# DeliriumV01D/NeRFpp

Measured on AMD Instinct MI355X. Metric: ray-samples/sec (HIP volume-rendering path, Lego 800x800, N_samples=64+128), higher is better.
Workload: dtype f16x3

## Files before the change

include/nerfpp_hip.h:

```cpp
#ifndef NERFPP_HIP_H
#define NERFPP_HIP_H

#include <stddef.h>
#include <stdint.h>

#ifdef __cplusplus
extern "C" {
#endif

#define NRF_API __attribute__((visibility("default")))

enum {
    NRF_OK = 0,
    NRF_ERR_INVALID_ARG = 1,
    NRF_ERR_HIP = 2,
    NRF_ERR_UNSUPPORTED = 3,
    NRF_ERR_WORKSPACE = 4,
    NRF_ERR_NONFINITE = 5
};

NRF_API int nrf_version(void);
NRF_API const char *nrf_last_error(void);
NRF_API const char *nrf_status_string(int status);

// ... 436 lines not shown
                                   void *d_workspace, size_t workspace_bytes, void *stream);
NRF_API size_t nrf_lerf_backward_points_workspace_bytes(const nrf_lerf_renderer *r, int64_t n, int s);
NRF_API int nrf_lerf_backward_points(const nrf_lerf_renderer *r, const float *d_pts, const float *d_z, const float *d_dirs, int d_stride, int64_t n, int s, const float *d_noise,
                                     float noise_std, const float *d_g_rendered, float *d_g_lerf_params, float *d_g_table, void *d_workspace, size_t workspace_bytes, void *stream);
NRF_API int nrf_lerf_renderer_last_features(const nrf_lerf_renderer *r, const void **d_feats_lm, int64_t *cols, const uint8_t **d_keep_cols, const int32_t **d_src, int64_t *n, int *sf,
                                            uint64_t *serial );
NRF_API int nrf_lerf_backward_points_src(const nrf_lerf_renderer *r, const void *d_feats_lm, int64_t cols, const uint8_t *d_keep_cols, const int32_t *d_src, const float *d_pts,
                                         const float *d_z, const float *d_dirs, int d_stride, int64_t n, int s, const float *d_noise, float noise_std, const float *d_g_rendered,
                                         float *d_g_lerf_params, float *d_g_table, void *d_workspace, size_t workspace_bytes, void *stream);

NRF_API size_t nrf_scratch_trim(void);

enum { NRF_PROF_HASH = 0, NRF_PROF_MLP = 1, NRF_PROF_COMPOSITE = 2, NRF_PROF_SAMPLE = 3, NRF_PROF_OTHER = 4, NRF_PROF_SIGMA = 5, NRF_PROF_MLP_COLOUR = 6, NRF_PROF_COUNT = 7 };
NRF_API int nrf_set_render_lanes(int lanes);
NRF_API int nrf_get_render_lanes(void);
NRF_API int nrf_renderer_set_lanes(nrf_renderer *r, int lanes);
NRF_API int nrf_fp32_gemm_available(void);
NRF_API int nrf_get_train_gemm(void);
NRF_API int nrf_set_train_gemm(int mode);
NRF_API int nrf_gemm_nt_bf16x3(const float *d_a, int lda, int64_t m, int k, const float *d_b, int ldb, int n, float *d_c, int ldc, const float *d_bias, int relu, void *stream);
NRF_API int nrf_gemm_tn_bf16x3(const float *d_g, int ldg, int out, const float *d_x, int ldx, int n, int64_t p, float *d_dw, int in, int col0, void *stream);
NRF_API int nrf_layer_grad_split(const float *d_g, int ldg, int out, const float *d_x, int ldx, int n, int64_t p, float *d_dw, int in, int col0, float *d_db, void *stream);
NRF_API int nrf_gemm_nt_f16x3(const float *d_a, int lda, int64_t m, int k, const float *d_b, int ldb, int n, float *d_c, int ldc, const float *d_bias, int relu, void *stream);
NRF_API int nrf_profile_enable(int on);
NRF_API int nrf_profile_is_enabled(void);
NRF_API int nrf_profile_read(double *ms , int64_t *launches , int reset);

#ifdef __cplusplus
}
#endif
// ... 2 lines not shown
```

nerfpp_amd/_lib.py:

```python
import ctypes as C
import os
import re

_HERE = os.path.dirname(os.path.abspath(__file__))
LIB_PATH = os.environ.get("NRF_LIB_PATH") or os.path.join(_HERE, "lib", "libnerfpp_hip.so")

NRF_OK = 0
NRF_HASH_NGP, NRF_HASH_CU = 0, 1
NRF_SH_LIBTORCH, NRF_SH_CUDA = 0, 1
NRF_PREC_F32, NRF_PREC_F16_MFMA, NRF_PREC_F16_SPLIT = 0, 1, 2
NRF_DIRS_NONE, NRF_DIRS_PE, NRF_DIRS_SH_LIBTORCH, NRF_DIRS_SH_CUDA = 0, 1, 2, 3
(NRF_RNG_T_RAND, NRF_RNG_R_COARSE, NRF_RNG_THETA_COARSE, NRF_RNG_NOISE_COARSE, NRF_RNG_U_PDF, NRF_RNG_PRECOND, NRF_RNG_R_FINE, NRF_RNG_THETA_FINE,
 NRF_RNG_NOISE_FINE) = range(1, 10)
NRF_PROF_NAMES = ("hash", "mlp", "composite", "sample", "other", "sigma", "mlp_colour")
NRF_COARSE_AUTO, NRF_COARSE_FULL, NRF_COARSE_SIGMA_F32 = 0, 1, 2
NRF_OVERFLOW_AUTO, NRF_OVERFLOW_RERENDER, NRF_OVERFLOW_ERROR, NRF_OVERFLOW_DEFERRED, NRF_OVERFLOW_IGNORE = 0, 1, 2, 3, 4
NRF_ERR_NONFINITE = 5
NRF_NORMALS_DENSITY, NRF_NORMALS_PREDICTED = 1, 2


class HashDesc(C.Structure):
    _fields_ = [("mode", C.c_int), ("n_levels", C.c_int), ("n_features", C.c_int), ("log2_hashmap_size", C.c_int),
                ("base_resolution", C.c_int), ("finest_resolution", C.c_int), ("bbox", C.c_float * 6)]

# ... 227 lines not shown
    nrf_lerf_head_relevancy(pplpipiiipppzp)
    nrf_lerf_point_relevancy_workspace_bytes(plil)->z
    nrf_lerf_point_relevancy(ppliipplpzp)
    nrf_lerf_relevancy_grid_workspace_bytes(piiiil)->z
    nrf_lerf_relevancy_grid(ppiiiiipplpzp)
    nrf_huber_rows_nanmean(pplifppp)
    nrf_lerf_head_backward_workspace_bytes(pli)->z
    nrf_lerf_head_backward(pppppilipfppppppzp)
    nrf_lerf_backward_points_workspace_bytes(pli)->z
    nrf_lerf_backward_points(ppppilipfppppzp)
    nrf_lerf_renderer_last_features(pppppppp)
    nrf_lerf_backward_points_src(pplpppppilipfppppzp)
    nrf_scratch_trim()->z
    nrf_set_render_lanes(i)
    nrf_get_render_lanes()
    nrf_renderer_set_lanes(pi)
    nrf_fp32_gemm_available()
    nrf_get_train_gemm()
    nrf_set_train_gemm(i)
    nrf_gemm_nt_bf16x3(pilipiipipip)
    nrf_gemm_tn_bf16x3(piipiilpiip)
    nrf_layer_grad_split(piipiilpiipp)
    nrf_gemm_nt_f16x3(pilipiipipip)
    nrf_profile_enable(i)
    nrf_profile_is_enabled()
    nrf_profile_read(ppi)
"""
SIGNATURES = {}
for _entry in _ABI.split():
    _m = re.fullmatch(r"(nrf_\w+)\(([ilzfduqp]*)\)(?:->([lzpsv]))?", _entry)
# ... 33 lines not shown
```

nerfpp_amd/csrc/mlp.h:

```cpp
#pragma once
#include "common.h"

#include <functional>
#include <vector>

namespace nrf {

enum { MLP_SMALL = 0, MLP_NERF = 1, MLP_LERF = 2 };

enum : uint8_t { WM_ZERO = 0, WM_F16_HI = 1, WM_F16_LO = 2, WM_F32 = 3 };
struct WeightMap {
    int32_t *d_src = nullptr;
    uint8_t *d_kind = nullptr;
    int64_t n = 0;
    int elem = 2;
    void *d_out = nullptr;
    bool scaled = false;
};

enum { SMALL_MAX_GROUPS = 12, SMALL_SCALE_INV_SIGMA = 0, SMALL_SCALE_INV_RGB = 1, SMALL_SCALE_HIDDEN = 2, SMALL_SCALE_COUNT = 8 };

struct LinearLayer {
    int in = 0, out = 0;
    float *d_wt = nullptr;
// ... 75 lines not shown
int train_gemm_mode();
int train_gemm_for(const nrf_mlp *m);
bool run_backprop_uses_mask_bits(const nrf_mlp *m, int64_t npts, int width);
bool gemm_nt_bits_ok(int64_t M, int N);
int gemm_nt_split(int arithmetic, int64_t M, int N, Seg a, Seg b, const float *B, int ldb, float *c, int ldc, const float *bias, int relu, const float *mask, int mask_ld,
                  hipStream_t st, const float *add = nullptr, int add_ld = 0, const float *r1s = nullptr, int r1s_ld = 0, const float *r1w = nullptr,
                  uint64_t *bits_out = nullptr, int bits_out_ld = 0, const uint64_t *bits_in = nullptr, int bits_in_ld = 0);
int gemm_rm(hipStream_t st, bool transA, bool transB, int64_t M, int64_t N, int64_t K, float alpha, const float *A, int lda, const float *B, int ldb, float beta, float *C, int ldc);

int mlp_small_mfma_available(const nrf_mlp *m);
int mlp_small_rescale(nrf_mlp *m, hipStream_t st);
int mlp_small_forward_mfma_lm(const nrf_mlp *m, const __half2 *feats, const __half2 *feats_lo, int64_t pstride, const __half *dirs, const __half *dirs_lo, int s,
                              const uint8_t *keep, int64_t p, float *out, hipStream_t st, const int32_t *src = nullptr);
int mlp_small_color_from_geo_lm(const nrf_mlp *m, const void *geo, int64_t geo_stride, const float *sigma, const __half *dirs, const __half *dirs_lo, int s,
                                const uint8_t *keep, int64_t p, float *out, hipStream_t st);
int mlp_small_pack_sigma_f32(nrf_mlp *m, const std::vector<float> &host_params);
int mlp_small_sigma_f32_available(const nrf_mlp *m);
int mlp_small_sigma_f32_lm(const nrf_mlp *m, const void *feats, int f32_in, int64_t pstride, const uint8_t *keep, int64_t p, float *sigma, hipStream_t st, void *geo = nullptr,
                           int64_t geo_stride = 0);
int mlp_nerf_mfma_available(const nrf_mlp *m);
int mlp_nerf_forward_mfma_fused(const nrf_mlp *m, const float *pts, const float *rays, int ray_stride, const float *z, int s, const __half *dirs, int64_t p, float *out, hipStream_t st);
int launch_dirs_pe_f16(const float *rays, int stride, int64_t n, __half *out, hipStream_t st);
int mlp_nerf_split_available(const nrf_mlp *m);
int mlp_nerf_forward_split_rows(const nrf_mlp *m, const float *x, int xs, int64_t p, float *out, int os, hipStream_t st);
int mlp_nerf_forward_split_fused(const nrf_mlp *m, const float *pts, const float *rays, int ray_stride, const float *z, int s, const __half *dirs, const __half *dirs_lo,
                                 int64_t p, float *out, hipStream_t st);
int launch_dirs_pe_split(const float *rays, int stride, int64_t n, __half *out_hi, __half *out_lo, hipStream_t st);
int mlp_small_pack_f16(nrf_mlp *m, const std::vector<float> &host_params);
int mlp_small_pack_bwd(nrf_mlp *m, const std::vector<float> &host_params);
bool mlp_small_images_host(const nrf_mlp_small_desc &d, const std::vector<float> &hp, std::vector<uint8_t> &f16_img, std::vector<uint8_t> &split_img);
// ... 25 lines not shown
```

nerfpp_amd/csrc/mlp_small_mfma.hip:

```cpp
#include "mfma_frag.h"
#include "mlp.h"

#include <type_traits>

namespace nrf {

typedef _Float16 half2v __attribute__((ext_vector_type(2)));

#ifdef NRF_SMALL_TRACE
__device__ unsigned long long g_small_trace[256 * 12];
#define NRF_TSTAMP(i) do { const unsigned long long t__ = __builtin_readcyclecounter(); tr[i] += t__ - tprev; tprev = t__; } while (0)
#else
#define NRF_TSTAMP(i) do { } while (0)
#endif
#ifndef NRF_SMALL_PT
#define NRF_SMALL_PT 2
#endif
constexpr int PT = NRF_SMALL_PT;
#ifndef NRF_SPLIT_WAVES
#define NRF_SPLIT_WAVES 8
#endif
#ifndef NRF_SPLIT_MINWAVES
#define NRF_SPLIT_MINWAVES 1
#endif
// ... 84 lines not shown
struct SmallPlan {
    static constexpr int GEO_KS = 1;
    static constexpr int sigma_frags(int l) { return (l == NL - 1 ? 1 : 2) * (l == 0 ? IN_KS : 4); }
    static constexpr int color_frags(int l) { return (l == NLC - 1 ? 1 : 2) * (l == 0 ? (V_KS + GEO_KS) : 4); }
    static constexpr int sigma_total() { int t = 0; for (int l = 0; l < NL; l++) t += sigma_frags(l); return t; }
    static constexpr int total()
    {
        int t = 0;
        for (int l = 0; l < NL; l++) t += sigma_frags(l);
        for (int l = 0; l < NLC; l++) t += color_frags(l);
        return t;
    }
};

struct SmallInput {
    const float *x; int x_stride; int in_ch;
    const __half2 *feats; int64_t pstride;
    const __half *dirs; int s;
    const uint8_t *keep;
    const __half *dirs_lo;
    const __half2 *feats_lo;
    const int32_t *src;
    const half8 *geo; int64_t geo_stride;
    const float *sigma;
    uint32_t ray_mul; int ray_shift;
    const float *scales;
};

#ifndef NRF_SMALL_PIPE_SPLIT
#define NRF_SMALL_PIPE_SPLIT 1
#endif
// ... 5 lines not shown
#endif
#ifndef NRF_SMALL_PREFETCH_F16
#define NRF_SMALL_PREFETCH_F16 0
#endif
#ifndef NRF_SMALL_STAGGER
#define NRF_SMALL_STAGGER 0
#endif
#ifndef NRF_SMALL_FINE
#define NRF_SMALL_FINE 1
#endif
#ifndef NRF_SMALL_DROP_MASK
#define NRF_SMALL_DROP_MASK 0
#endif
constexpr int small_drop_of(int id) { return (int)((((unsigned long long)NRF_SMALL_DROP_MASK) >> (2 * id)) & 3ull); }

template <int IN_KS, int V_KS, int NL, int NLC, bool LM, bool SPLIT, bool LMLO = false, bool GEOIN = false, bool A32 = false>
__global__ void __launch_bounds__(64 * waves_of(SPLIT), SPLIT ? NRF_SPLIT_MINWAVES : 2)
k_mlp_small_mfma(int64_t npts, SmallInput in, const half8 *__restrict__ packed, float *__restrict__ out, int out_stride)
{
    using Plan = SmallPlan<IN_KS, V_KS, NL, NLC>;
    constexpr int NP = SPLIT ? 2 : 1;
    constexpr int BLOCK_PTS = block_pts_of(SPLIT);
    constexpr bool IN_LO = SPLIT && (!LM || LMLO);
    static_assert(!GEOIN || (LM && SPLIT && !LMLO), "the colour-only kernel exists in split precision on the level-major path");
    extern __shared__ __attribute__((aligned(16))) unsigned char smem[];
    half8 *wl = reinterpret_cast<half8 *>(smem);
    constexpr int NFRAG = Plan::total() * NP;
    for (int i = threadIdx.x; i < NFRAG * 64; i += blockDim.x) wl[i] = packed[i];
    __syncthreads();

    const int lane = threadIdx.x & 63, wave = threadIdx.x >> 6;
    const int r = lane & 31, h = lane >> 5;
    const int64_t nblocks = (npts + BLOCK_PTS - 1) / BLOCK_PTS;
    float inv_sigma = 1.0f, inv_rgb = 1.0f;
    if constexpr (SPLIT) { inv_sigma = in.scales[SMALL_SCALE_INV_SIGMA]; inv_rgb = in.scales[SMALL_SCALE_INV_RGB]; }
    (void)inv_sigma; (void)inv_rgb;
#if NRF_SMALL_STAGGER
    if (SPLIT && wave >= 4) {
#pragma unroll
        for (int i = 0; i < NRF_SMALL_STAGGER; i++) __builtin_amdgcn_s_sleep(127);
    }
#endif
    auto split8 = [](const float4 &lo4, const float4 &hi4, half8 &hv, half8 &lv) {
        const float v[8] = {lo4.x, lo4.y, lo4.z, lo4.w, hi4.x, hi4.y, hi4.z, hi4.w};
#pragma unroll
        for (int j = 0; j < 8; j++) { const _Float16 t = (_Float16)v[j]; hv[j] = t; lv[j] = (_Float16)(v[j] - (float)t); }
    };
    static_assert(!A32 || (LM && SPLIT), "32-bit addressing is instantiated for the split-precision level-major kernels");
    auto load_cols = [&](int64_t blk_, int32_t (&cols)[PT]) {
        if (A32 || !(LM && in.src)) return;
        const int64_t p0_ = blk_ * BLOCK_PTS + wave * (32 * PT);
#pragma unroll
        for (int pt = 0; pt < PT; pt++) {
            int64_t p = p0_ + pt * 32 + r;
            if (p >= npts) p = npts - 1;
            cols[pt] = (LM && in.src) ? in.src[p] : (int32_t)0;
        }
    };
    auto load_inputs = [&](int64_t blk_, const int32_t (&cols)[PT], half8 (&bx)[PT][IN_KS][NP], half8 (&bv)[PT][V_KS][NP], uint8_t (&kpv)[PT], half8 (&bg)[PT][NP], float (&sgv)[PT]) {
        const int64_t p0_ = blk_ * BLOCK_PTS + wave * (32 * PT);
#pragma unroll
        for (int pt = 0; pt < PT; pt++) {
            int64_t p = p0_ + pt * 32 + r;
            if (p >= npts) p = npts - 1;
            kpv[pt] = 1;
            if constexpr (LM) {
                if constexpr (A32) {
                    uint32_t pu = (uint32_t)p0_ + (uint32_t)(pt * 32 + r);
                    pu = pu < (uint32_t)npts ? pu : (uint32_t)npts - 1u;
                    if (in.keep) kpv[pt] = in.keep[pu];
                    if constexpr (GEOIN) {
                        const uint32_t goff = (pu * 2u + (uint32_t)h) * 16u;
                        bg[pt][0] = *reinterpret_cast<const half8 *>(reinterpret_cast<const char *>(in.geo) + goff);
                        bg[pt][NP - 1] = *reinterpret_cast<const half8 *>(reinterpret_cast<const char *>(in.geo + in.geo_stride * 2) + goff);
                        sgv[pt] = in.sigma[pu];
                    } else {
                        const uint32_t voff = ((uint32_t)(4 * h) * (uint32_t)in.pstride + pu) * 4u;
#pragma unroll
                        for (int s = 0; s < IN_KS; s++) {
                            union { half8 v; __half2 q[4]; } u;
#pragma unroll
                            for (int q = 0; q < 4; q++) u.q[q] = *reinterpret_cast<const __half2 *>(reinterpret_cast<const char *>(in.feats + (int64_t)(8 * s + q) * in.pstride) + voff);
                            bx[pt][s][0] = u.v;
                            if constexpr (SPLIT && LMLO) {
#pragma unroll
// ... 45 lines not shown
                    const float4 hi = *reinterpret_cast<const float4 *>(row + 16 * s + 8 * h + 4);
                    if constexpr (SPLIT) split8(lo, hi, bx[pt][s][0], bx[pt][s][NP - 1]);
                    else bx[pt][s][0] = half8{(_Float16)lo.x, (_Float16)lo.y, (_Float16)lo.z, (_Float16)lo.w, (_Float16)hi.x, (_Float16)hi.y, (_Float16)hi.z, (_Float16)hi.w};
                }
#pragma unroll
                for (int s = 0; s < V_KS; s++) {
                    const float4 lo = *reinterpret_cast<const float4 *>(row + in.in_ch + 16 * s + 8 * h);
                    const float4 hi = *reinterpret_cast<const float4 *>(row + in.in_ch + 16 * s + 8 * h + 4);
                    if constexpr (SPLIT) split8(lo, hi, bv[pt][s][0], bv[pt][s][NP - 1]);
                    else bv[pt][s][0] = half8{(_Float16)lo.x, (_Float16)lo.y, (_Float16)lo.z, (_Float16)lo.w, (_Float16)hi.x, (_Float16)hi.y, (_Float16)hi.z, (_Float16)hi.w};
                }
            }
        }
    };
    constexpr bool PREFETCH = LM && (SPLIT ? (NRF_SMALL_PREFETCH_SPLIT != 0) : (NRF_SMALL_PREFETCH_F16 != 0));
    half8 bx[PT][IN_KS][NP];
    half8 bv[PT][V_KS][NP];
    half8 bxn[PREFETCH ? PT : 1][IN_KS][NP];
    half8 bvn[PREFETCH ? PT : 1][V_KS][NP];
    half8 bg[PT][NP], bgn[PT][NP];
    float sgv[PT], sgn[PT];
    (void)bg; (void)bgn; (void)sgv; (void)sgn;
    uint8_t kp[PT], kpn[PT];
    int32_t cols_next[PT];
#pragma unroll
    for (int pt = 0; pt < PT; pt++) { kp[pt] = 1; kpn[pt] = 1; cols_next[pt] = 0; }
    if constexpr (PREFETCH) {
        if ((int64_t)blockIdx.x < nblocks) {
            int32_t c0[PT];
            load_cols(blockIdx.x, c0);
            if ((int64_t)blockIdx.x + gridDim.x < nblocks) load_cols((int64_t)blockIdx.x + gridDim.x, cols_next);
            load_inputs(blockIdx.x, c0, bx, bv, kp, bg, sgv);
        }
    }
#ifdef NRF_SMALL_TRACE
    unsigned long long tr[12] = {0, 0, 0, 0, 0, 0, 0, 0, 0, 0, 0, 0};
#endif
    for (int64_t blk = blockIdx.x; blk < nblocks; blk += gridDim.x) {
#ifdef NRF_SMALL_TRACE
        const unsigned long long titer = __builtin_readcyclecounter();
        unsigned long long tprev = titer;
#endif
        const int64_t p0 = blk * BLOCK_PTS + wave * (32 * PT);
        if constexpr (!PREFETCH) { int32_t c0[PT]; load_cols(blk, c0); load_inputs(blk, c0, bx, bv, kp, bg, sgv); }
        const bool more = blk + gridDim.x < nblocks;
        const half8 *fr = wl;
        constexpr bool PIPE = SPLIT ? (NRF_SMALL_PIPE_SPLIT != 0) : (NRF_SMALL_PIPE_F16 != 0);
// ... 90 lines not shown
                                if (i >= i0 && i < i1) conv_item(bb, tt, i);
                        }
                    }
                }
            };
        };
        if constexpr (GEOIN) fr += Plan::sigma_total() * 64 * NP;
        half8 pre[NP];
#pragma unroll
        for (int q = 0; q < NP; q++) pre[q] = fr[q * 64 + lane];
        f32x16 sig[PT][1];
        auto prefetch_next = [&]() {
            if constexpr (PREFETCH) {
                if (more) {
                    load_inputs(blk + gridDim.x, cols_next, bxn, bvn, kpn, bgn, sgn);
                    if (blk + 2 * (int64_t)gridDim.x < nblocks) load_cols(blk + 2 * (int64_t)gridDim.x, cols_next);
                }
            }
        };
        if constexpr (GEOIN) {
        } else if constexpr (NL == 1) {
            gemm_layer<1, IN_KS, NP, IN_LO>(fr, lane, bx, sig, pre); fr += Plan::sigma_frags(0) * 64 * NP;
        } else {
            gemm_layer<2, IN_KS, NP, IN_LO, false, FINE, small_drop_of(0)>(fr, lane, bx, acc2, pre, make_job(1, false, true, IN_KS, std::true_type{}, std::bool_constant<!(small_drop_of(1) & 2)>{})); fr += Plan::sigma_frags(0) * 64 * NP;
            prefetch_next();
            NRF_TSTAMP(0);
            static_assert(NL <= 3, "sigma net: at most three layers");
            if constexpr (NL == 3) {
                if constexpr (!PIPE) hidden_to_b(0);
                gemm_layer<2, 4, NP, SPLIT, false, FINE, small_drop_of(1)>(fr, lane, bh[0], acc2, pre, make_job(0, true, true, 4, std::bool_constant<!(small_drop_of(1) & 2)>{}, std::bool_constant<!(small_drop_of(2) & 2)>{}));
// ... 42 lines not shown
                fr += Plan::color_frags(2) * 64 * NP;
                NRF_TSTAMP(6);
            }
            {
                constexpr int l = NLC - 1;
                const int bi = PIPE ? ((l - 1) & 1) : 0;
                if constexpr (!PIPE) hidden_to_b(0);
                gemm_layer<1, 4, NP, SPLIT, true, FINE, small_drop_of(NL + l)>(fr, lane, bh[bi], rgb, pre, make_job(bi, true, false, 4, std::bool_constant<!(small_drop_of(NL + l) & 2)>{}, std::true_type{}));
                fr += Plan::color_frags(l) * 64 * NP;
                NRF_TSTAMP(4 + l);
            }
        }
        if (h == 0) {
#pragma unroll
            for (int pt = 0; pt < PT; pt++) {
                const int64_t p = p0 + pt * 32 + r;
                if (p < npts) {
                    float sg;
                    if constexpr (GEOIN) sg = sgv[pt]; else if constexpr (SPLIT) sg = sig[pt][0][0] * inv_sigma; else sg = sig[pt][0][0];
                    if constexpr (LM) { if (!kp[pt]) sg = 0.0f; }
                    float c0 = rgb[pt][0][0], c1 = rgb[pt][0][1], c2 = rgb[pt][0][2];
                    if constexpr (SPLIT) { c0 *= inv_rgb; c1 *= inv_rgb; c2 *= inv_rgb; }
                    if (out_stride == 4) *reinterpret_cast<float4 *>(out + p * 4) = float4{c0, c1, c2, sg};
                    else { float *o = out + p * out_stride; o[0] = c0; o[1] = c1; o[2] = c2; o[3] = sg; }
                }
            }
        }
        if constexpr (PREFETCH) {
            if (more) {
#pragma unroll
                for (int pt = 0; pt < PT; pt++) {
#pragma unroll
                    for (int s = 0; s < IN_KS; s++)
#pragma unroll
                        for (int q = 0; q < NP; q++) bx[pt][s][q] = bxn[pt][s][q];
#pragma unroll
                    for (int s = 0; s < V_KS; s++)
#pragma unroll
                        for (int q = 0; q < NP; q++) bv[pt][s][q] = bvn[pt][s][q];
                    kp[pt] = kpn[pt];
                    if constexpr (GEOIN) { bg[pt][0] = bgn[pt][0]; bg[pt][NP - 1] = bgn[pt][NP - 1]; sgv[pt] = sgn[pt]; }
                }
            }
        }
#ifdef NRF_SMALL_TRACE
        NRF_TSTAMP(8);
        tr[9] += __builtin_readcyclecounter() - titer; tr[10] += 1;
#endif
    }
#ifdef NRF_SMALL_TRACE
    if (threadIdx.x == 0 && SPLIT && LM) for (int i = 0; i < 12; i++) g_small_trace[blockIdx.x * 12 + i] += tr[i];
#endif
}

#ifdef NRF_SMALL_TRACE
extern "C" NRF_API int nrf_dbg_small_trace(unsigned long long *host_out, int reset)
// ... 80 lines not shown
    if (!mlp_small_images_host(d, hp, a, b)) return NRF_OK;
    auto upload = [](void *&dst, size_t &have, const std::vector<uint8_t> &img) -> int {
        const size_t bytes = img.size();
        if (dst && have != bytes) { (void)hipFree(dst); dst = nullptr; }
        if (!dst) NRF_HIP(hipMalloc(&dst, bytes));
        have = bytes;
        NRF_HIP(hipMemcpy(dst, img.data(), bytes, hipMemcpyHostToDevice));
        return NRF_OK;
    };
    NRF_TRY(upload(m->d_packed_f16, m->packed_f16_bytes, a));
    NRF_TRY(upload(m->d_packed_split, m->packed_split_bytes, b));
    return mlp_small_pack_bwd(m, hp);
}

template <int V_KS, int NL, int NLC>
static int launch_small(const nrf_mlp *m, const SmallInput &in, bool lm, bool split, int64_t p, float *out, int os, hipStream_t st)
{
    using Plan = SmallPlan<2, V_KS, NL, NLC>;
    const size_t lds = (size_t)Plan::total() * 1024 * (split ? 2 : 1);
    const size_t have = split ? m->packed_split_bytes : m->packed_f16_bytes;
    if (lds != have) { set_error("internal: packed weight image is %zu bytes, kernel expects %zu", have, lds); return NRF_ERR_INVALID_ARG; }
    const int64_t nblocks = ceil_div(p, block_pts_of(split));
    const int64_t cap = split ? 256 : 768;
    const unsigned grid = (unsigned)(nblocks < cap ? nblocks : cap);
    const half8 *img = reinterpret_cast<const half8 *>(split ? m->d_packed_split : m->d_packed_f16);
#define NRF_GO(LM_, SP_, LO_, ...)                                                                                                            \
    do {                                                                                                                                      \
        auto kfn = k_mlp_small_mfma<2, V_KS, NL, NLC, LM_, SP_, LO_, ##__VA_ARGS__>;                                                          \
        if (lds > 64 * 1024) NRF_HIP(hipFuncSetAttribute(reinterpret_cast<const void *>(kfn), hipFuncAttributeMaxDynamicSharedMemorySize, (int)lds)); \
        hipLaunchKernelGGL(kfn, dim3(grid), dim3(64 * waves_of(SP_)), lds, st, p, in, img, out, os);                                          \
    } while (0)
    const bool a32 = lm && split && !in.src && (p >> 26) == 0 && (in.pstride >> 27) == 0 && (in.geo_stride >> 26) == 0 && in.ray_mul != 0 &&
                     (((uint64_t)(p / (in.s > 0 ? in.s : 1)) + 1) * (uint64_t)(32 * V_KS)) >> 32 == 0;
    if (in.geo) {
        if (!lm || !split) { set_error("internal: the colour-only NeRFSmall kernel is split precision, level-major"); return NRF_ERR_INVALID_ARG; }
        if (a32) NRF_GO(true, true, false, true, true); else NRF_GO(true, true, false, true);
    } else if (lm) {
        if (split) {
            if (in.feats_lo) { if (a32) NRF_GO(true, true, true, false, true); else NRF_GO(true, true, true); }
            else { if (a32) NRF_GO(true, true, false, false, true); else NRF_GO(true, true, false); }
        } else NRF_GO(true, false, false);
    }
    else { if (split) NRF_GO(false, true, false); else NRF_GO(false, false, false); }
#undef NRF_GO
    NRF_LAUNCH_CHECK();
    return NRF_OK;
}

static int dispatch_small(const nrf_mlp *m, const SmallInput &in, bool lm, bool split, int64_t p, float *out, int os, hipStream_t st);

int mlp_small_mfma_available(const nrf_mlp *m) { return m && m->family == MLP_SMALL && m->d_packed_f16 != nullptr && m->d_packed_split != nullptr; }

int mlp_small_forward_mfma_lm(const nrf_mlp *m, const __half2 *feats, const __half2 *feats_lo, int64_t pstride, const __half *dirs, const __half *dirs_lo, int s,
                              const uint8_t *keep, int64_t p, float *out, hipStream_t st, const int32_t *src)
{
    if (!mlp_small_mfma_available(m)) { set_error("internal: matrix-core NeRFSmall image missing"); return NRF_ERR_UNSUPPORTED; }
    ProfScope prof(NRF_PROF_MLP, st);
    SmallInput in{nullptr, 0, m->small.input_ch, feats, pstride, dirs, s, keep, dirs_lo, dirs_lo ? feats_lo : nullptr, src, nullptr, 0, nullptr};
    return dispatch_small(m, in, true, dirs_lo != nullptr, p, out, 4, st);
}

int mlp_small_color_from_geo_lm(const nrf_mlp *m, const void *geo, int64_t geo_stride, const float *sigma, const __half *dirs, const __half *dirs_lo, int s,
                                const uint8_t *keep, int64_t p, float *out, hipStream_t st)
{
    if (!mlp_small_mfma_available(m)) { set_error("internal: matrix-core NeRFSmall image missing"); return NRF_ERR_UNSUPPORTED; }
    if (!geo || !sigma || !dirs_lo) { set_error("internal: colour-only pass without geo planes / sigma / split direction features"); return NRF_ERR_INVALID_ARG; }
    ProfScope prof(NRF_PROF_MLP_COLOUR, st);
    SmallInput in{nullptr, 0, m->small.input_ch, nullptr, 0, dirs, s, keep, dirs_lo, nullptr, nullptr, static_cast<const half8 *>(geo), geo_stride, sigma};
    return dispatch_small(m, in, true, true, p, out, 4, st);
}

int mlp_small_forward_mfma(const nrf_mlp *m, const float *x, int xs, int64_t p, int split, float *out, int os, hipStream_t st)
{
    const auto &d = m->small;
    if (!m->d_packed_f16) {
        set_error("NRF_PREC_F16_MFMA / NRF_PREC_F16_SPLIT: NeRFSmall shape (in %d, views %d, %dx%d, geo %d, colour %dx%d) is outside the built matrix-core family; use NRF_PREC_F32",
                  d.input_ch, d.input_ch_views, d.num_layers, d.hidden_dim, d.geo_feat_dim, d.num_layers_color, d.hidden_dim_color);
        return NRF_ERR_UNSUPPORTED;
    }
    if ((xs % 4) != 0 || (reinterpret_cast<uintptr_t>(x) & 15)) { set_error("NRF_PREC_F16_MFMA: input rows must be 16-byte aligned"); return NRF_ERR_INVALID_ARG; }
    SmallInput in{x, xs, d.input_ch, nullptr, 0, nullptr, 1, nullptr, nullptr, nullptr, nullptr, nullptr, 0, nullptr};
    return dispatch_small(m, in, false, split != 0, p, out, os, st);
}

static int dispatch_small(const nrf_mlp *m, const SmallInput &in_, bool lm, bool split, int64_t p, float *out, int os, hipStream_t st)
{
    const auto &d = m->small;
    SmallInput in = in_;
    in.ray_mul = 0; in.ray_shift = 0;
    in.scales = m->d_scales;
    if (lm && in.s >= 1) {
        int L = 0;
        while ((1 << L) < in.s) L++;
        if (L == 0) { in.ray_mul = 1; in.ray_shift = -1; }
        else { in.ray_mul = (uint32_t)((((uint64_t)1 << (31 + L)) + (uint64_t)in.s - 1) / (uint64_t)in.s); in.ray_shift = L - 1; }
    }
    const int v = d.input_ch_views / 16;
#define NRF_CASE(V, NL, NLC) if (v == V && d.num_layers == NL && d.num_layers_color == NLC) return launch_small<V, NL, NLC>(m, in, lm, split, p, out, os, st);
    NRF_CASE(1, 3, 4) NRF_CASE(1, 3, 3) NRF_CASE(1, 3, 2) NRF_CASE(1, 2, 4) NRF_CASE(1, 2, 3) NRF_CASE(1, 2, 2)
    NRF_CASE(4, 3, 4) NRF_CASE(4, 3, 3) NRF_CASE(4, 3, 2) NRF_CASE(4, 2, 4) NRF_CASE(4, 2, 3) NRF_CASE(4, 2, 2)
#undef NRF_CASE
    set_error("internal: no matrix-core instantiation for this NeRFSmall shape");
    return NRF_ERR_UNSUPPORTED;
}

}
```

nerfpp_amd/csrc/render.hip:

```cpp
#include "chunk_loop.h"
#include "encode.h"
#include "hash_fast.h"
#include "mlp.h"
#include "stoch.h"

#include <atomic>
#include <cstdlib>
#include <mutex>

struct nrf_renderer {
    nrf_renderer_desc desc;
    int in_ch = 0, in_views = 0;
    mutable nrf::Lanes chunk_lanes;
    int lanes = 0;
    mutable uint32_t *d_flags = nullptr, *h_flags = nullptr, *h_deferred = nullptr;
    mutable hipEvent_t deferred_ev[32] = {};
    mutable int deferred_slots[32] = {};
    mutable int deferred_head = 0;
    mutable int64_t flagged_chunks = 0, rerendered_chunks = 0;
    mutable nrf::FeatureView view;
    ~nrf_renderer()
    {
        chunk_lanes.drop();
        for (auto &e : deferred_ev) if (e) { (void)hipEventSynchronize(e); (void)hipEventDestroy(e); }
// ... 366 lines not shown
    a.exact_classic = ni > 0 && a.fast_classic && mlp_nerf_sigma_f32_available(r->desc.mlp) && c == 4 &&
                      (p->coarse_mode == NRF_COARSE_SIGMA_F32 || (p->coarse_mode == NRF_COARSE_AUTO && a.classic_split));
    a.split = a.fast && p->precision == NRF_PREC_F16_SPLIT;
    a.ngp = a.fast && r->desc.hash->desc.mode == NRF_HASH_NGP;
    a.reuse_raw = (a.fast || a.fast_classic) && ni > 0 && !a.sigma_only && !cone && !precond && c == 4 && n * (int64_t)sf < ((int64_t)1 << 31);
    a.reuse = !a.reuse_raw && a.fast && ni > 0 && !cone && !precond && n * (int64_t)sf < ((int64_t)1 << 31);
    a.geo_reuse = a.reuse && a.sigma_only && a.split && r->desc.mlp->small.geo_feat_dim <= 15;
    return a;
}

struct PathWs {
    NetWs net;
    FastWs fw;
    ReuseWs rw;
    void *geo_planes; float *raw_cols;
    int32_t *rr_src; float *rr_znew, *rr_rawnew;
};
static PathWs path_layout(Bump &b, const nrf_renderer *r, const Path &a, int64_t n, int s, int ni, int prec)
{
    PathWs w{};
    const int sf = s + ni;
    const int64_t pmax = n * (int64_t)(a.reuse_raw ? (s > ni ? s : ni) : sf);
    if (a.reuse) {
        w.rw = reuse_layout(b, n, s, ni, a.ngp && a.split, a.ngp && a.sigma_only);
        if (a.geo_reuse) { w.geo_planes = b.take<char>((size_t)n * s * 64); w.raw_cols = b.take<float>((size_t)n * sf * 4); }
    } else if (a.fast) w.fw = fast_layout(b, r, pmax);
    else if (!a.fast_classic) w.net = network_layout(b, r, pmax, prec);
    if (a.reuse_raw) {
        w.rr_src = b.take<int32_t>((size_t)n * sf);
        w.rr_znew = b.take<float>((size_t)n * ni);
        w.rr_rawnew = b.take<float>((size_t)n * ni * 4);
    }
    return w;
}

struct ChunkWs {
    float *z_c, *w_c, *raw_c, *z_f, *raw_f;
    __half *dirs16, *dirs_lo;
    float *z_plain;
    float *pts;
// ... 290 lines not shown
    if (path.reuse_raw) {
        PointSource psn{nullptr, d_rays, pw.rr_znew, ray_stride, ni};
        NRF_TRY(network(psn, ni, pw.rr_rawnew));
        if (out->d_raw) {
            hipLaunchKernelGGL(k_gather_raw, dim3((unsigned)ceil_div(n * (int64_t)sf, 256)), dim3(256), 0, st, n * (int64_t)sf, pw.rr_src, reinterpret_cast<const float4 *>(cw.raw_c),
                               reinterpret_cast<const float4 *>(pw.rr_rawnew), n * (int64_t)s, reinterpret_cast<float4 *>(cw.raw_f));
            NRF_LAUNCH_CHECK();
        } else { raw_final = cw.raw_c; raw2_final = pw.rr_rawnew; split_final = n * (int64_t)s; src_final = pw.rr_src; }
    } else if (path.reuse) {
        PointSource psn{nullptr, d_rays, rw.z_new, ray_stride, ni};
        if (path.ngp) NRF_TRY(launch_hash_ngp_lm(r->desc.hash, psn, n * (int64_t)ni, rw.feats + n * (int64_t)s, rw.cols, rw.feats_lo ? rw.feats_lo - rw.feats : 0, rw.keep + n * (int64_t)s, st));
        else NRF_TRY(launch_hash_lm(r->desc.hash, psn, n * (int64_t)ni, rw.feats + n * (int64_t)s, rw.cols, rw.keep + n * (int64_t)s, HASH_LM_DEFAULT_VARIANT, st));
        if (!path.ngp) r->view.set(rw.feats, rw.cols, rw.keep, rw.src, n, sf);
        if (path.geo_reuse) {
            const int64_t nc = n * (int64_t)s;
            NRF_TRY(mlp_small_color_from_geo_lm(r->desc.mlp, pw.geo_planes, nc, cw.raw_c, cw.dirs16, cw.dirs_lo, s, rw.keep, nc, pw.raw_cols, st));
            NRF_TRY(mlp_small_forward_mfma_lm(r->desc.mlp, rw.feats + nc, rw.feats_lo ? rw.feats_lo + nc : nullptr, rw.cols, cw.dirs16, cw.dirs_lo, ni, rw.keep + nc, n * (int64_t)ni,
                                              pw.raw_cols + nc * 4, st));
            if (out->d_raw) {
                hipLaunchKernelGGL(k_gather_raw, dim3((unsigned)ceil_div(n * (int64_t)sf, 256)), dim3(256), 0, st, n * (int64_t)sf, rw.src, reinterpret_cast<const float4 *>(pw.raw_cols),
                                   reinterpret_cast<const float4 *>(pw.raw_cols) + nc, nc, reinterpret_cast<float4 *>(cw.raw_f));
                NRF_LAUNCH_CHECK();
            } else { raw_final = pw.raw_cols; src_final = rw.src; }
        } else NRF_TRY(mlp_small_forward_mfma_lm(r->desc.mlp, rw.feats, rw.feats_lo, rw.cols, cw.dirs16, cw.dirs_lo, sf, rw.keep, n * (int64_t)sf, cw.raw_f, st, rw.src));
    } else NRF_TRY(network(psf, sf, cw.raw_f));
    nz.stream = NRF_RNG_NOISE_FINE;
    float *w_final = out->d_weights ? out->d_weights : cw.nrm_w;
    NRF_TRY(launch_raw2outputs(raw_final, cw.z_f, d_rays + 3, ray_stride, n, sf, c, 3, p->white_bkgr, out->d_rgb, out->d_disp, out->d_acc,
                               w_final, out->d_depth, nz, st, fastc, src_final, raw2_final, split_final, d_flag));
    return p->normals ? normals_tail(psf, w_final, cw.raw_f) : NRF_OK;
}
// ... 366 lines not shown
```

Baseline: 7.459 billion.

## Compact live coarse points and run colour MLP only where sigma is positive

Adds a three-kernel stream compaction (per-block count, single-block scan, scatter) that lists coarse samples with sigma > 0. For dead samples it writes zero colour rows directly. A new list-mode instantiation of the colour-only split-precision MFMA kernel then gathers geo planes only for listed points and exits early past the device-side count. This skips colour MLP work in empty space, at the cost of extra compaction launches, a serial single-block scan, and indirect gathers. It is on by default and falls back to the full pass when noise is on or raw outputs are requested.

```diff
diff --git a/include/nerfpp_hip.h b/include/nerfpp_hip.h
--- a/include/nerfpp_hip.h
+++ b/include/nerfpp_hip.h
@@ -474,6 +474,10 @@
 enum { NRF_PROF_HASH = 0, NRF_PROF_MLP = 1, NRF_PROF_COMPOSITE = 2, NRF_PROF_SAMPLE = 3, NRF_PROF_OTHER = 4, NRF_PROF_SIGMA = 5, NRF_PROF_MLP_COLOUR = 6, NRF_PROF_COUNT = 7 };
 NRF_API int nrf_set_render_lanes(int lanes);
 NRF_API int nrf_get_render_lanes(void);
+NRF_API int nrf_set_live_colour(int on);
+NRF_API int nrf_get_live_colour(void);
+NRF_API size_t nrf_live_points_workspace_bytes(int64_t p);
+NRF_API int nrf_live_points(const float *d_sigma, int64_t p, int32_t *d_list, int32_t *d_count, float *d_raw_rows, void *d_workspace, size_t workspace_bytes, void *stream);
 NRF_API int nrf_renderer_set_lanes(nrf_renderer *r, int lanes);
 NRF_API int nrf_fp32_gemm_available(void);
 NRF_API int nrf_get_train_gemm(void);
diff --git a/nerfpp_amd/_lib.py b/nerfpp_amd/_lib.py
--- a/nerfpp_amd/_lib.py
+++ b/nerfpp_amd/_lib.py
@@ -265,6 +265,10 @@
     nrf_scratch_trim()->z
     nrf_set_render_lanes(i)
     nrf_get_render_lanes()
+    nrf_set_live_colour(i)
+    nrf_get_live_colour()
+    nrf_live_points_workspace_bytes(l)->z
+    nrf_live_points(plppppzp)
     nrf_renderer_set_lanes(pi)
     nrf_fp32_gemm_available()
     nrf_get_train_gemm()
diff --git a/nerfpp_amd/csrc/live_points.h b/nerfpp_amd/csrc/live_points.h
--- /dev/null
+++ b/nerfpp_amd/csrc/live_points.h
@@ -0,0 +1,14 @@
+#pragma once
+
+#include "workspace.h"
+
+namespace nrf {
+
+struct LiveWs {
+    int32_t *sums;
+};
+LiveWs live_points_layout(Bump &b, int64_t p);
+int live_points_launch(const float *sigma, int64_t p, int32_t *list, int32_t *count, float *rows, const LiveWs &w, hipStream_t st);
+int live_colour_on();
+
+}
diff --git a/nerfpp_amd/csrc/live_points.hip b/nerfpp_amd/csrc/live_points.hip
--- /dev/null
+++ b/nerfpp_amd/csrc/live_points.hip
@@ -0,0 +1,145 @@
+#include "live_points.h"
+#include "scan.h"
+
+namespace nrf {
+
+constexpr int LIVE_WAVES = 4, LIVE_STEPS = 8;
+constexpr int LIVE_BLOCK_PTS = 64 * LIVE_STEPS * LIVE_WAVES;
+constexpr int LIVE_SCAN_B = 1024;
+
+static inline int64_t live_blocks(int64_t p) { return ceil_div(p, LIVE_BLOCK_PTS); }
+
+__device__ __forceinline__ void live_load(const float *__restrict__ sigma, uint32_t p0, uint32_t p, int lane, float (&sg)[LIVE_STEPS])
+{
+#pragma unroll
+    for (int k = 0; k < LIVE_STEPS; k++) {
+        const uint32_t i = p0 + (uint32_t)(k * 64 + lane);
+        sg[k] = i < p ? sigma[i] : 0.0f;
+    }
+}
+
+__global__ void __launch_bounds__(64 * LIVE_WAVES)
+k_live_count(uint32_t p, const float *__restrict__ sigma, int32_t *__restrict__ sums)
+{
+    __shared__ int32_t wsum[LIVE_WAVES];
+    const int lane = threadIdx.x & 63, wave = threadIdx.x >> 6;
+    float sg[LIVE_STEPS];
+    live_load(sigma, blockIdx.x * (uint32_t)LIVE_BLOCK_PTS + (uint32_t)(wave * 64 * LIVE_STEPS), p, lane, sg);
+    int32_t c = 0;
+#pragma unroll
+    for (int k = 0; k < LIVE_STEPS; k++) c += __popcll(__ballot(sg[k] > 0.0f));
+    if (lane == 0) wsum[wave] = c;
+    __syncthreads();
+    if (threadIdx.x == 0) {
+        int32_t t = 0;
+#pragma unroll
+        for (int w = 0; w < LIVE_WAVES; w++) t += wsum[w];
+        sums[blockIdx.x] = t;
+    }
+}
+
+__global__ void __launch_bounds__(LIVE_SCAN_B)
+k_live_scan(int32_t nb, int32_t *__restrict__ sums, int32_t *__restrict__ count)
+{
+    __shared__ int32_t sh[LIVE_SCAN_B];
+    int32_t carry = 0;
+    for (int32_t base = 0; base < nb; base += LIVE_SCAN_B) {
+        const int32_t i = base + (int32_t)threadIdx.x;
+        const int32_t v = i < nb ? sums[i] : 0;
+        int32_t total;
+        const int32_t ex = block_exclusive_scan<int32_t, LIVE_SCAN_B>(v, sh, total);
+        if (i < nb) sums[i] = carry + ex;
+        carry += total;
+        __syncthreads();
+    }
+    if (threadIdx.x == 0) *count = carry;
+}
+
+__global__ void __launch_bounds__(64 * LIVE_WAVES)
+k_live_scatter(uint32_t p, const float *__restrict__ sigma, const int32_t *__restrict__ sums, int32_t *__restrict__ list, float4 *__restrict__ rows)
+{
+    __shared__ int32_t wsum[LIVE_WAVES];
+    const int lane = threadIdx.x & 63, wave = threadIdx.x >> 6;
+    const uint32_t p0 = blockIdx.x * (uint32_t)LIVE_BLOCK_PTS + (uint32_t)(wave * 64 * LIVE_STEPS);
+    float sg[LIVE_STEPS];
+    live_load(sigma, p0, p, lane, sg);
+    uint64_t mask[LIVE_STEPS];
+    int32_t c = 0;
+#pragma unroll
+    for (int k = 0; k < LIVE_STEPS; k++) { mask[k] = __ballot(sg[k] > 0.0f); c += __popcll(mask[k]); }
+    if (lane == 0) wsum[wave] = c;
+    __syncthreads();
+    int32_t at = sums[blockIdx.x];
+    for (int w = 0; w < wave; w++) at += wsum[w];
+    const uint64_t below = (1ull << lane) - 1ull;
+#pragma unroll
+    for (int k = 0; k < LIVE_STEPS; k++) {
+        const uint32_t i = p0 + (uint32_t)(k * 64 + lane);
+        if ((mask[k] >> lane) & 1ull) list[at + __popcll(mask[k] & below)] = (int32_t)i;
+        else if (rows && i < p) rows[i] = float4{0.0f, 0.0f, 0.0f, sg[k]};
+        at += __popcll(mask[k]);
+    }
+}
+
+LiveWs live_points_layout(Bump &b, int64_t p)
+{
+    LiveWs w{};
+    w.sums = b.take<int32_t>((size_t)live_blocks(p));
+    return w;
+}
+
+int live_points_launch(const float *sigma, int64_t p, int32_t *list, int32_t *count, float *rows, const LiveWs &w, hipStream_t st)
+{
+    if (p <= 0 || p >= ((int64_t)1 << 31)) { set_error("internal: live-point compaction of %lld points (1 .. 2^31 - 1)", (long long)p); return NRF_ERR_INVALID_ARG; }
+    const unsigned nb = (unsigned)live_blocks(p);
+    hipLaunchKernelGGL(k_live_count, dim3(nb), dim3(64 * LIVE_WAVES), 0, st, (uint32_t)p, sigma, w.sums);
+    hipLaunchKernelGGL(k_live_scan, dim3(1), dim3(LIVE_SCAN_B), 0, st, (int32_t)nb, w.sums, count);
+    hipLaunchKernelGGL(k_live_scatter, dim3(nb), dim3(64 * LIVE_WAVES), 0, st, (uint32_t)p, sigma, w.sums, list, reinterpret_cast<float4 *>(rows));
+    NRF_LAUNCH_CHECK();
+    return NRF_OK;
+}
+
+static std::atomic<int> g_live_colour{-1};
+int live_colour_on()
+{
+    int v = g_live_colour.load(std::memory_order_relaxed);
+    if (v < 0) {
+        const char *e = getenv("NRF_LIVE_COLOUR");
+        v = (e && strcmp(e, "0") == 0) ? 0 : 1;
+        g_live_colour.store(v, std::memory_order_relaxed);
+    }
+    return v;
+}
+
+}
+
+extern "C" {
+
+int nrf_set_live_colour(int on)
+{
+    NRF_CHECK_ARG(on == 0 || on == 1, "nrf_set_live_colour: 0 (colour at every coarse depth) or 1 (only where sigma > 0)");
+    nrf::g_live_colour.store(on, std::memory_order_relaxed);
+    return NRF_OK;
+}
+
+int nrf_get_live_colour(void) { return nrf::live_colour_on(); }
+
+size_t nrf_live_points_workspace_bytes(int64_t p)
+{
+    if (p <= 0) return 0;
+    return nrf::measure([&](nrf::Bump &b) { nrf::live_points_layout(b, p); });
+}
+
+int nrf_live_points(const float *d_sigma, int64_t p, int32_t *d_list, int32_t *d_count, float *d_raw_rows, void *d_workspace, size_t workspace_bytes, void *stream)
+{
+    NRF_CHECK_ARG(d_sigma && d_list && d_count, "nrf_live_points: null pointer");
+    NRF_CHECK_ARG(p >= 1 && p < ((int64_t)1 << 31), "nrf_live_points: 1 <= p < 2^31 points");
+    NRF_CHECK_ARG(!d_raw_rows || (reinterpret_cast<uintptr_t>(d_raw_rows) & 15) == 0, "nrf_live_points: d_raw_rows must be 16-byte aligned");
+    NRF_CHECK_ARG(d_workspace, "nrf_live_points: null workspace");
+    nrf::Bump bump(d_workspace, workspace_bytes);
+    const nrf::LiveWs w = nrf::live_points_layout(bump, p);
+    NRF_TRY(nrf::ws_check(bump, nrf_live_points_workspace_bytes(p), "nrf_live_points"));
+    return nrf::live_points_launch(d_sigma, p, d_list, d_count, d_raw_rows, w, nrf::as_stream(stream));
+}
+
+}
diff --git a/nerfpp_amd/csrc/mlp.h b/nerfpp_amd/csrc/mlp.h
--- a/nerfpp_amd/csrc/mlp.h
+++ b/nerfpp_amd/csrc/mlp.h
@@ -113,6 +113,9 @@
                               const uint8_t *keep, int64_t p, float *out, hipStream_t st, const int32_t *src = nullptr);
 int mlp_small_color_from_geo_lm(const nrf_mlp *m, const void *geo, int64_t geo_stride, const float *sigma, const __half *dirs, const __half *dirs_lo, int s,
                                 const uint8_t *keep, int64_t p, float *out, hipStream_t st);
+bool mlp_small_color_list_ok(const nrf_mlp *m, int64_t p, int s);
+int mlp_small_color_from_geo_list_lm(const nrf_mlp *m, const void *geo, int64_t geo_stride, const float *sigma, const __half *dirs, const __half *dirs_lo, int s,
+                                     int64_t p, const int32_t *list, const int32_t *count, float *out, hipStream_t st);
 int mlp_small_pack_sigma_f32(nrf_mlp *m, const std::vector<float> &host_params);
 int mlp_small_sigma_f32_available(const nrf_mlp *m);
 int mlp_small_sigma_f32_lm(const nrf_mlp *m, const void *feats, int f32_in, int64_t pstride, const uint8_t *keep, int64_t p, float *sigma, hipStream_t st, void *geo = nullptr,
diff --git a/nerfpp_amd/csrc/mlp_small_mfma.hip b/nerfpp_amd/csrc/mlp_small_mfma.hip
--- a/nerfpp_amd/csrc/mlp_small_mfma.hip
+++ b/nerfpp_amd/csrc/mlp_small_mfma.hip
@@ -122,7 +122,8 @@
 };
 
 struct SmallInput {
-    const float *x; int x_stride; int in_ch;
+    union { const float *x; const int32_t *count; };
+    int x_stride; int in_ch;
     const __half2 *feats; int64_t pstride;
     const __half *dirs; int s;
     const uint8_t *keep;
@@ -158,11 +159,17 @@
 #endif
 constexpr int small_drop_of(int id) { return (int)((((unsigned long long)NRF_SMALL_DROP_MASK) >> (2 * id)) & 3ull); }
 
-template <int IN_KS, int V_KS, int NL, int NLC, bool LM, bool SPLIT, bool LMLO = false, bool GEOIN = false, bool A32 = false>
+template <int IN_KS, int V_KS, int NL, int NLC, bool LM, bool SPLIT, bool LMLO = false, bool GEOIN = false, bool A32 = false, bool LIST = false>
 __global__ void __launch_bounds__(64 * waves_of(SPLIT), SPLIT ? NRF_SPLIT_MINWAVES : 2)
 k_mlp_small_mfma(int64_t npts, SmallInput in, const half8 *__restrict__ packed, float *__restrict__ out, int out_stride)
 {
     using Plan = SmallPlan<IN_KS, V_KS, NL, NLC>;
+    static_assert(!LIST || (GEOIN && A32), "the list mode exists for the colour-only kernel with 32-bit addressing");
+    if constexpr (LIST) {
+        const int32_t cnt = *in.count;
+        npts = cnt < npts ? cnt : npts;
+        if ((int64_t)blockIdx.x * block_pts_of(SPLIT) >= npts) return;
+    }
     constexpr int NP = SPLIT ? 2 : 1;
     constexpr int BLOCK_PTS = block_pts_of(SPLIT);
     constexpr bool IN_LO = SPLIT && (!LM || LMLO);
@@ -192,6 +199,16 @@
     };
     static_assert(!A32 || (LM && SPLIT), "32-bit addressing is instantiated for the split-precision level-major kernels");
     auto load_cols = [&](int64_t blk_, int32_t (&cols)[PT]) {
+        if constexpr (LIST) {
+            const uint32_t q0 = (uint32_t)blk_ * (uint32_t)BLOCK_PTS + (uint32_t)(wave * (32 * PT));
+#pragma unroll
+            for (int pt = 0; pt < PT; pt++) {
+                uint32_t q = q0 + (uint32_t)(pt * 32 + r);
+                q = q < (uint32_t)npts ? q : (uint32_t)npts - 1u;
+                cols[pt] = in.src[q];
+            }
+            return;
+        }
         if (A32 || !(LM && in.src)) return;
         const int64_t p0_ = blk_ * BLOCK_PTS + wave * (32 * PT);
 #pragma unroll
@@ -212,7 +229,8 @@
                 if constexpr (A32) {
                     uint32_t pu = (uint32_t)p0_ + (uint32_t)(pt * 32 + r);
                     pu = pu < (uint32_t)npts ? pu : (uint32_t)npts - 1u;
-                    if (in.keep) kpv[pt] = in.keep[pu];
+                    if constexpr (LIST) pu = (uint32_t)cols[pt];
+                    else if (in.keep) kpv[pt] = in.keep[pu];
                     if constexpr (GEOIN) {
                         const uint32_t goff = (pu * 2u + (uint32_t)h) * 16u;
                         bg[pt][0] = *reinterpret_cast<const half8 *>(reinterpret_cast<const char *>(in.geo) + goff);
@@ -288,6 +306,7 @@
         }
     };
     constexpr bool PREFETCH = LM && (SPLIT ? (NRF_SMALL_PREFETCH_SPLIT != 0) : (NRF_SMALL_PREFETCH_F16 != 0));
+    static_assert(!LIST || PREFETCH, "the list mode hands its columns over with the prefetched operands");
     half8 bx[PT][IN_KS][NP];
     half8 bv[PT][V_KS][NP];
     half8 bxn[PREFETCH ? PT : 1][IN_KS][NP];
@@ -297,14 +316,20 @@
     (void)bg; (void)bgn; (void)sgv; (void)sgn;
     uint8_t kp[PT], kpn[PT];
     int32_t cols_next[PT];
-#pragma unroll
-    for (int pt = 0; pt < PT; pt++) { kp[pt] = 1; kpn[pt] = 1; cols_next[pt] = 0; }
+    int32_t cols_cur[PT], cols_pre[PT];
+    (void)cols_cur; (void)cols_pre;
+#pragma unroll
+    for (int pt = 0; pt < PT; pt++) { kp[pt] = 1; kpn[pt] = 1; cols_next[pt] = 0; cols_cur[pt] = 0; cols_pre[pt] = 0; }
     if constexpr (PREFETCH) {
         if ((int64_t)blockIdx.x < nblocks) {
             int32_t c0[PT];
             load_cols(blockIdx.x, c0);
             if ((int64_t)blockIdx.x + gridDim.x < nblocks) load_cols((int64_t)blockIdx.x + gridDim.x, cols_next);
             load_inputs(blockIdx.x, c0, bx, bv, kp, bg, sgv);
+            if constexpr (LIST) {
+#pragma unroll
+                for (int pt = 0; pt < PT; pt++) cols_cur[pt] = c0[pt];
+            }
         }
     }
 #ifdef NRF_SMALL_TRACE
@@ -425,6 +450,10 @@
             if constexpr (PREFETCH) {
                 if (more) {
                     load_inputs(blk + gridDim.x, cols_next, bxn, bvn, kpn, bgn, sgn);
+                    if constexpr (LIST) {
+#pragma unroll
+                        for (int pt = 0; pt < PT; pt++) cols_pre[pt] = cols_next[pt];
+                    }
                     if (blk + 2 * (int64_t)gridDim.x < nblocks) load_cols(blk + 2 * (int64_t)gridDim.x, cols_next);
                 }
             }
@@ -497,8 +526,9 @@
         if (h == 0) {
 #pragma unroll
             for (int pt = 0; pt < PT; pt++) {
-                const int64_t p = p0 + pt * 32 + r;
+                int64_t p = p0 + pt * 32 + r;
                 if (p < npts) {
+                    if constexpr (LIST) p = cols_cur[pt];
                     float sg;
                     if constexpr (GEOIN) sg = sgv[pt]; else if constexpr (SPLIT) sg = sig[pt][0][0] * inv_sigma; else sg = sig[pt][0][0];
                     if constexpr (LM) { if (!kp[pt]) sg = 0.0f; }
@@ -523,6 +553,7 @@
                         for (int q = 0; q < NP; q++) bv[pt][s][q] = bvn[pt][s][q];
                     kp[pt] = kpn[pt];
                     if constexpr (GEOIN) { bg[pt][0] = bgn[pt][0]; bg[pt][NP - 1] = bgn[pt][NP - 1]; sgv[pt] = sgn[pt]; }
+                    if constexpr (LIST) cols_cur[pt] = cols_pre[pt];
                 }
             }
         }
@@ -633,7 +664,7 @@
 }
 
 template <int V_KS, int NL, int NLC>
-static int launch_small(const nrf_mlp *m, const SmallInput &in, bool lm, bool split, int64_t p, float *out, int os, hipStream_t st)
+static int launch_small(const nrf_mlp *m, const SmallInput &in, bool lm, bool split, int64_t p, float *out, int os, hipStream_t st, bool listed)
 {
     using Plan = SmallPlan<2, V_KS, NL, NLC>;
     const size_t lds = (size_t)Plan::total() * 1024 * (split ? 2 : 1);
@@ -649,11 +680,14 @@
         if (lds > 64 * 1024) NRF_HIP(hipFuncSetAttribute(reinterpret_cast<const void *>(kfn), hipFuncAttributeMaxDynamicSharedMemorySize, (int)lds)); \
         hipLaunchKernelGGL(kfn, dim3(grid), dim3(64 * waves_of(SP_)), lds, st, p, in, img, out, os);                                          \
     } while (0)
-    const bool a32 = lm && split && !in.src && (p >> 26) == 0 && (in.pstride >> 27) == 0 && (in.geo_stride >> 26) == 0 && in.ray_mul != 0 &&
+    const bool a32 = lm && split && (!in.src || listed) && (p >> 26) == 0 && (in.pstride >> 27) == 0 && (in.geo_stride >> 26) == 0 && in.ray_mul != 0 &&
                      (((uint64_t)(p / (in.s > 0 ? in.s : 1)) + 1) * (uint64_t)(32 * V_KS)) >> 32 == 0;
     if (in.geo) {
         if (!lm || !split) { set_error("internal: the colour-only NeRFSmall kernel is split precision, level-major"); return NRF_ERR_INVALID_ARG; }
-        if (a32) NRF_GO(true, true, false, true, true); else NRF_GO(true, true, false, true);
+        if (listed) {
+            if (!a32 || !in.src || !in.count) { set_error("internal: the listed colour-only launch needs 32-bit addressing ranges (%lld points)", (long long)p); return NRF_ERR_INVALID_ARG; }
+            NRF_GO(true, true, false, true, true, true);
+        } else if (a32) NRF_GO(true, true, false, true, true); else NRF_GO(true, true, false, true);
     } else if (lm) {
         if (split) {
             if (in.feats_lo) { if (a32) NRF_GO(true, true, true, false, true); else NRF_GO(true, true, true); }
@@ -666,7 +700,7 @@
     return NRF_OK;
 }
 
-static int dispatch_small(const nrf_mlp *m, const SmallInput &in, bool lm, bool split, int64_t p, float *out, int os, hipStream_t st);
+static int dispatch_small(const nrf_mlp *m, const SmallInput &in, bool lm, bool split, int64_t p, float *out, int os, hipStream_t st, bool listed = false);
 
 int mlp_small_mfma_available(const nrf_mlp *m) { return m && m->family == MLP_SMALL && m->d_packed_f16 != nullptr && m->d_packed_split != nullptr; }
 
@@ -675,7 +709,7 @@
 {
     if (!mlp_small_mfma_available(m)) { set_error("internal: matrix-core NeRFSmall image missing"); return NRF_ERR_UNSUPPORTED; }
     ProfScope prof(NRF_PROF_MLP, st);
-    SmallInput in{nullptr, 0, m->small.input_ch, feats, pstride, dirs, s, keep, dirs_lo, dirs_lo ? feats_lo : nullptr, src, nullptr, 0, nullptr};
+    SmallInput in{{nullptr}, 0, m->small.input_ch, feats, pstride, dirs, s, keep, dirs_lo, dirs_lo ? feats_lo : nullptr, src, nullptr, 0, nullptr};
     return dispatch_small(m, in, true, dirs_lo != nullptr, p, out, 4, st);
 }
 
@@ -685,8 +719,24 @@
     if (!mlp_small_mfma_available(m)) { set_error("internal: matrix-core NeRFSmall image missing"); return NRF_ERR_UNSUPPORTED; }
     if (!geo || !sigma || !dirs_lo) { set_error("internal: colour-only pass without geo planes / sigma / split direction features"); return NRF_ERR_INVALID_ARG; }
     ProfScope prof(NRF_PROF_MLP_COLOUR, st);
-    SmallInput in{nullptr, 0, m->small.input_ch, nullptr, 0, dirs, s, keep, dirs_lo, nullptr, nullptr, static_cast<const half8 *>(geo), geo_stride, sigma};
+    SmallInput in{{nullptr}, 0, m->small.input_ch, nullptr, 0, dirs, s, keep, dirs_lo, nullptr, nullptr, static_cast<const half8 *>(geo), geo_stride, sigma};
     return dispatch_small(m, in, true, true, p, out, 4, st);
+}
+
+bool mlp_small_color_list_ok(const nrf_mlp *m, int64_t p, int s)
+{
+    const int v_ks = m->small.input_ch_views / 16;
+    return s >= 1 && p >= 1 && (p >> 26) == 0 && (((uint64_t)(p / s) + 1) * (uint64_t)(32 * v_ks)) >> 32 == 0;
+}
+
+int mlp_small_color_from_geo_list_lm(const nrf_mlp *m, const void *geo, int64_t geo_stride, const float *sigma, const __half *dirs, const __half *dirs_lo, int s,
+                                     int64_t p, const int32_t *list, const int32_t *count, float *out, hipStream_t st)
+{
+    if (!mlp_small_mfma_available(m)) { set_error("internal: matrix-core NeRFSmall image missing"); return NRF_ERR_UNSUPPORTED; }
+    if (!geo || !sigma || !dirs_lo || !list || !count) { set_error("internal: listed colour-only pass without geo planes / sigma / split direction features / list"); return NRF_ERR_INVALID_ARG; }
+    SmallInput in{{nullptr}, 0, m->small.input_ch, nullptr, 0, dirs, s, nullptr, dirs_lo, nullptr, list, static_cast<const half8 *>(geo), geo_stride, sigma};
+    in.count = count;
+    return dispatch_small(m, in, true, true, p, out, 4, st, true);
 }
 
 int mlp_small_forward_mfma(const nrf_mlp *m, const float *x, int xs, int64_t p, int split, float *out, int os, hipStream_t st)
@@ -698,11 +748,11 @@
         return NRF_ERR_UNSUPPORTED;
     }
     if ((xs % 4) != 0 || (reinterpret_cast<uintptr_t>(x) & 15)) { set_error("NRF_PREC_F16_MFMA: input rows must be 16-byte aligned"); return NRF_ERR_INVALID_ARG; }
-    SmallInput in{x, xs, d.input_ch, nullptr, 0, nullptr, 1, nullptr, nullptr, nullptr, nullptr, nullptr, 0, nullptr};
+    SmallInput in{{x}, xs, d.input_ch, nullptr, 0, nullptr, 1, nullptr, nullptr, nullptr, nullptr, nullptr, 0, nullptr};
     return dispatch_small(m, in, false, split != 0, p, out, os, st);
 }
 
-static int dispatch_small(const nrf_mlp *m, const SmallInput &in_, bool lm, bool split, int64_t p, float *out, int os, hipStream_t st)
+static int dispatch_small(const nrf_mlp *m, const SmallInput &in_, bool lm, bool split, int64_t p, float *out, int os, hipStream_t st, bool listed)
 {
     const auto &d = m->small;
     SmallInput in = in_;
@@ -715,7 +765,7 @@
         else { in.ray_mul = (uint32_t)((((uint64_t)1 << (31 + L)) + (uint64_t)in.s - 1) / (uint64_t)in.s); in.ray_shift = L - 1; }
     }
     const int v = d.input_ch_views / 16;
-#define NRF_CASE(V, NL, NLC) if (v == V && d.num_layers == NL && d.num_layers_color == NLC) return launch_small<V, NL, NLC>(m, in, lm, split, p, out, os, st);
+#define NRF_CASE(V, NL, NLC) if (v == V && d.num_layers == NL && d.num_layers_color == NLC) return launch_small<V, NL, NLC>(m, in, lm, split, p, out, os, st, listed);
     NRF_CASE(1, 3, 4) NRF_CASE(1, 3, 3) NRF_CASE(1, 3, 2) NRF_CASE(1, 2, 4) NRF_CASE(1, 2, 3) NRF_CASE(1, 2, 2)
     NRF_CASE(4, 3, 4) NRF_CASE(4, 3, 3) NRF_CASE(4, 3, 2) NRF_CASE(4, 2, 4) NRF_CASE(4, 2, 3) NRF_CASE(4, 2, 2)
 #undef NRF_CASE
diff --git a/nerfpp_amd/csrc/render.hip b/nerfpp_amd/csrc/render.hip
--- a/nerfpp_amd/csrc/render.hip
+++ b/nerfpp_amd/csrc/render.hip
@@ -1,6 +1,7 @@
 #include "chunk_loop.h"
 #include "encode.h"
 #include "hash_fast.h"
+#include "live_points.h"
 #include "mlp.h"
 #include "stoch.h"
 
@@ -404,6 +405,7 @@
     FastWs fw;
     ReuseWs rw;
     void *geo_planes; float *raw_cols;
+    int32_t *live_list, *live_count; LiveWs live;
     int32_t *rr_src; float *rr_znew, *rr_rawnew;
 };
 static PathWs path_layout(Bump &b, const nrf_renderer *r, const Path &a, int64_t n, int s, int ni, int prec)
@@ -413,7 +415,10 @@
     const int64_t pmax = n * (int64_t)(a.reuse_raw ? (s > ni ? s : ni) : sf);
     if (a.reuse) {
         w.rw = reuse_layout(b, n, s, ni, a.ngp && a.split, a.ngp && a.sigma_only);
-        if (a.geo_reuse) { w.geo_planes = b.take<char>((size_t)n * s * 64); w.raw_cols = b.take<float>((size_t)n * sf * 4); }
+        if (a.geo_reuse) {
+            w.geo_planes = b.take<char>((size_t)n * s * 64); w.raw_cols = b.take<float>((size_t)n * sf * 4);
+            w.live_list = b.take<int32_t>((size_t)n * s); w.live_count = b.take<int32_t>(1); w.live = live_points_layout(b, n * (int64_t)s);
+        }
     } else if (a.fast) w.fw = fast_layout(b, r, pmax);
     else if (!a.fast_classic) w.net = network_layout(b, r, pmax, prec);
     if (a.reuse_raw) {
@@ -734,7 +739,11 @@
         if (!path.ngp) r->view.set(rw.feats, rw.cols, rw.keep, rw.src, n, sf);
         if (path.geo_reuse) {
             const int64_t nc = n * (int64_t)s;
-            NRF_TRY(mlp_small_color_from_geo_lm(r->desc.mlp, pw.geo_planes, nc, cw.raw_c, cw.dirs16, cw.dirs_lo, s, rw.keep, nc, pw.raw_cols, st));
+            if (!out->d_raw && !nz.on && live_colour_on() && mlp_small_color_list_ok(r->desc.mlp, nc, s)) {
+                ProfScope prof(NRF_PROF_MLP_COLOUR, st);
+                NRF_TRY(live_points_launch(cw.raw_c, nc, pw.live_list, pw.live_count, pw.raw_cols, pw.live, st));
+                NRF_TRY(mlp_small_color_from_geo_list_lm(r->desc.mlp, pw.geo_planes, nc, cw.raw_c, cw.dirs16, cw.dirs_lo, s, nc, pw.live_list, pw.live_count, pw.raw_cols, st));
+            } else NRF_TRY(mlp_small_color_from_geo_lm(r->desc.mlp, pw.geo_planes, nc, cw.raw_c, cw.dirs16, cw.dirs_lo, s, rw.keep, nc, pw.raw_cols, st));
             NRF_TRY(mlp_small_forward_mfma_lm(r->desc.mlp, rw.feats + nc, rw.feats_lo ? rw.feats_lo + nc : nullptr, rw.cols, cw.dirs16, cw.dirs_lo, ni, rw.keep + nc, n * (int64_t)ni,
                                               pw.raw_cols + nc * 4, st));
             if (out->d_raw) {
```

New measurement: 7.602 billion (median of 6 runs). +1.9%, better.
